# wonjune-kang/llm-speech-summarization

Measured on AMD Instinct MI355X. Metric: generated tokens/s of end-to-end generate_audio_response steps (encode + prefill + 256-token greedy decode), HuBERT-large -> Llama-3.2-3B; audio-sec/s reported beside it, encoder stage alone and in the pipeline, higher is better.
Workload: dtype bf16

## Files before the change

include/speechllm.h:

```cpp
#ifndef SPEECHLLM_H
#define SPEECHLLM_H

#include <stddef.h>
#include <stdint.h>

#ifdef __cplusplus
extern "C" {
#endif

typedef void* sl_stream;

enum sl_dtype { SL_F32 = 0, SL_BF16 = 1, SL_F16 = 2 };
enum sl_status {
  SL_OK = 0,
  SL_ERR_ARG = -1,
  SL_ERR_LAUNCH = -2,
  SL_ERR_UNSUPPORTED = -3
};
enum sl_act { SL_ACT_NONE = 0, SL_ACT_GELU = 1, SL_ACT_SILU_MUL = 2, SL_ACT_ROPE_KV = 3 };
enum sl_w_layout { SL_W_ROWMAJOR = 0, SL_W_PACKED = 1 };
#define SL_W_PACKED_E4M3 2

const char* sl_last_error(void);
#define SL_ABI_VERSION 7
// ... 11 lines not shown
  int32_t dtype, act, out_f32, w_layout;
} sl_gemm_args;
int sl_gemm(const sl_gemm_args* a, sl_stream stream);

int sl_pack_weight(const void* src, int64_t ld_src, void* dst, int32_t N, int32_t K, int32_t dtype, sl_stream stream);

size_t sl_w8_image_bytes(int32_t N, int32_t K);
int sl_pack_weight_e4m3(const void* src, int64_t ld_src, void* dst, int32_t N, int32_t K, int32_t dtype, sl_stream stream);
int sl_pack_weight_e4m3_host(const void* src, int64_t ld_src, void* dst, int32_t N, int32_t K, int32_t dtype);
int32_t sl_w8_max_rows(void);

typedef struct {
  int32_t fuse_rms; float rms_eps;
  const float* rope_cos; const float* rope_sin;
  const int32_t* tok_pos; const int32_t* tok_seq;
  void* k_cache; void* v_cache;
  int32_t n_heads, n_kv_heads, max_ctx, reserved;
  void* split_ws; size_t split_ws_bytes;
  const float* rstd_in; float* rstd_out;
  void* norm_out; const void* norm_gain;
} sl_gemm_fused;
size_t sl_gemm_split_workspace_bytes(int32_t M, int32_t N, int32_t K, int32_t dtype);
int32_t sl_gemm_split_count(int32_t M, int32_t N, int32_t K, int32_t dtype);
int sl_gemm_fused_decode(const sl_gemm_args* a, const sl_gemm_fused* fx, sl_stream stream);

typedef struct {
  int32_t trans_a, trans_w, residual_f32, w_mod;
  void* aux_out;
  const int64_t* groups;
  int32_t groups_ext, reserved;
  float* amax_val; int32_t* amax_idx;
  const float* ln_mr; const float* ln_u; const float* ln_c; float* stats_out;
  void* sk_ws; size_t sk_ws_bytes;
  int32_t post_op, post_reserved;
  float drop_p; float post_reserved_f;
  uint64_t drop_seed;
  int64_t drop_ld;
  const void* post_in; int64_t post_ld;
  float* colsum_out;
  int32_t* deferred_splits;
} sl_gemm_ex_args;
enum { SL_POST_NONE = 0, SL_POST_DROPOUT = 1, SL_POST_GELU_BWD = 2, SL_POST_SILU_MUL_BWD = 3 };
int sl_gemm_ex(const sl_gemm_args* a, const sl_gemm_ex_args* ex, sl_stream stream);
size_t sl_gemm_streamk_workspace_bytes(void);
int32_t sl_gemm_ln_fold_ok(int32_t M, int32_t N, int32_t K, int32_t dtype);
int sl_layernorm_fold_build(const void* W, const void* gain, const void* beta, const void* bias, void* Wf, float* u, float* c, int32_t N,
// ... 411 lines not shown
```

llm-speech-summarization_amd/_lib.py:

```python
from __future__ import annotations

import ctypes as C
import os

import torch

_HERE = os.path.dirname(os.path.abspath(__file__))
LIB_PATH = (os.environ.get("SL_LIB_PATH") if os.environ.get("SL_DEV") == "1" else None) or os.path.join(_HERE, "libspeechllm.so")

SL_F32, SL_BF16, SL_F16 = 0, 1, 2
KV_MODEL_DTYPE, KV_FP8_E4M3 = 0, 1
ACT_NONE, ACT_GELU, ACT_SILU_MUL, ACT_ROPE_KV = 0, 1, 2, 3
POST_NONE, POST_DROPOUT, POST_GELU_BWD, POST_SILU_MUL_BWD = 0, 1, 2, 3
W_ROWMAJOR, W_PACKED, W_PACKED_E4M3 = 0, 1, 2
WDEC_MODEL_DTYPE, WDEC_E4M3 = 0, 1
COMM_ID_BYTES = 128
MAX_DECODE_BATCH = 2048

c_i32, c_i64, c_f32, c_vp, c_sz = C.c_int32, C.c_int64, C.c_float, C.c_void_p, C.c_size_t


class SpeechLLMError(RuntimeError):
    pass

# ... 163 lines not shown
    "sl_device_arch": (c_i32, [C.c_char_p, c_i32]),
    "sl_tuning_reload": (c_i32, []),
    "sl_decode_graph_cache_clear": (c_i32, []),
    "sl_gemm": (c_i32, [C.POINTER(GemmArgs), c_vp]),
    "sl_gemm_streamk_workspace_bytes": (C.c_size_t, []),
    "sl_layernorm_fold_build": (c_i32, [c_vp, c_vp, c_vp, c_vp, c_vp, c_vp, c_vp, c_i32, c_i32, c_i32, c_vp]),
    "sl_weight_norm_bwd": (c_i32, [c_vp, c_vp, c_vp, c_vp, c_vp, c_vp, c_i32, c_i32, c_i32, c_vp]),
    "sl_weight_norm_bwd_workspace_bytes": (C.c_size_t, [c_i32]),
    "sl_comm_unique_id": (c_i32, [c_vp]),
    "sl_comm_init": (c_i32, [C.POINTER(c_vp), c_vp, c_i32, c_i32]),
    "sl_allreduce_sum": (c_i32, [c_vp, c_vp, c_i64, c_i32, c_vp]),
    "sl_comm_destroy": (c_i32, [c_vp]),
    "sl_comm_abort": (c_i32, [c_vp]),
    "sl_comm_rank": (c_i32, [c_vp]),
    "sl_comm_world": (c_i32, [c_vp]),
    "sl_pack_weight": (c_i32, [c_vp, c_i64, c_vp, c_i32, c_i32, c_i32, c_vp]),
    "sl_w8_image_bytes": (c_sz, [c_i32, c_i32]),
    "sl_pack_weight_e4m3": (c_i32, [c_vp, c_i64, c_vp, c_i32, c_i32, c_i32, c_vp]),
    "sl_pack_weight_e4m3_host": (c_i32, [c_vp, c_i64, c_vp, c_i32, c_i32, c_i32]),
    "sl_w8_max_rows": (c_i32, []),
    "sl_gemm_fused_decode": (c_i32, [C.POINTER(GemmArgs), C.POINTER(GemmFused), c_vp]),
    "sl_gemm_split_workspace_bytes": (c_sz, [c_i32, c_i32, c_i32, c_i32]),
    "sl_gemm_split_count": (c_i32, [c_i32, c_i32, c_i32, c_i32]),
    "sl_attn_decode_workspace_bytes": (c_sz, [c_i32, c_i32, c_i32, c_i32]),
    "sl_attn_decode_split": (c_i32, [c_vp, c_i64, c_vp, c_vp, c_vp, c_vp, c_vp, c_i32, c_i32, c_i32, c_i32, c_i32, c_f32, c_i32, c_vp]),
    "sl_gemm_ex": (c_i32, [C.POINTER(GemmArgs), C.POINTER(GemmEx), c_vp]),
    "sl_gemm_ln_fold_ok": (c_i32, [c_i32, c_i32, c_i32, c_i32]),
    "sl_layernorm_stats_finalize": (c_i32, [c_vp, c_i32, c_i64, c_i32, c_f32, c_vp, c_vp]),
    "sl_layernorm_stats": (c_i32, [c_vp, c_i64, c_i32, c_f32, c_vp, c_i32, c_vp]),
    "sl_gelu_bwd": (c_i32, [c_vp, c_vp, c_vp, c_i64, c_i32, c_vp]),
    "sl_axpby": (c_i32, [c_vp, c_vp, c_f32, c_f32, c_i64, c_i32, c_vp]),
    "sl_adamw_blocks": (C.c_size_t, [c_i64]),
    "sl_adamw_step": (c_i32, [c_vp, c_vp, c_i32, c_i64, C.c_double, C.c_double, C.c_double, C.c_double, C.c_double, c_i64, c_vp]),
    "sl_attn_dropout_bwd": (c_i32, [c_vp, c_vp, c_vp, c_i64, c_i32, c_vp, c_i32, c_vp, c_i32, c_i32, c_i32, c_f32, C.c_uint64, c_i32, c_vp]),
    "sl_transpose_pad": (c_i32, [c_vp, c_i64, c_vp, c_i64, c_i32, c_i32, c_i32, c_i32, c_vp]),
    "sl_dropout": (c_i32, [c_vp, c_vp, c_vp, c_i64, c_f32, C.c_uint64, c_i32, c_vp]),
    "sl_silu_mul": (c_i32, [c_vp, c_vp, c_i64, c_i32, c_i32, c_vp]),
    "sl_silu_mul_bwd": (c_i32, [c_vp, c_vp, c_vp, c_i64, c_i32, c_i32, c_vp]),
    "sl_rope_inplace": (c_i32, [c_vp, c_vp, c_vp, c_vp, c_i64, c_i32, c_i32, c_i32, c_i32, c_i32, c_vp]),
    "sl_layernorm_bwd": (c_i32, [c_vp, c_vp, c_vp, c_vp, c_vp, c_vp, c_vp, c_i64, c_i32, c_f32, c_i32, c_i32, c_vp]),
    "sl_layernorm_bwd_ws_bytes": (c_sz, [c_i64, c_i32]),
    "sl_layernorm_bwd_ws": (c_i32, [c_vp, c_vp, c_vp, c_vp, c_vp, c_vp, c_vp, c_i64, c_i32, c_f32, c_i32, c_i32, c_vp, c_sz, c_vp]),
    "sl_rmsnorm_bwd": (c_i32, [c_vp, c_vp, c_vp, c_vp, c_i64, c_i32, c_f32, c_i32, c_vp]),
    "sl_colsum": (c_i32, [c_vp, c_i64, c_vp, c_i64, c_i32, c_i32, c_vp]),
    "sl_softmax_rows": (c_i32, [c_vp, c_vp, c_i64, c_i32, c_i32, c_i64, c_f32, c_i32, c_i32, c_vp]),
    "sl_softmax_bwd": (c_i32, [c_vp, c_vp, c_vp, c_i64, c_i32, c_i64, c_f32, c_i32, c_vp]),
# ... 168 lines not shown
```

llm-speech-summarization_amd/csrc/api.hip:

```cpp
#include <stdarg.h>
#include <stdlib.h>

#include <atomic>
#include <mutex>

#include "common.h"

static thread_local char g_err[512] = "";

void sl_set_error(const char* fmt, ...) {
  va_list ap;
  va_start(ap, fmt);
  vsnprintf(g_err, sizeof(g_err), fmt, ap);
  va_end(ap);
}

extern "C" const char* sl_last_error(void) { return g_err; }

extern "C" int sl_version(void) { return SL_ABI_VERSION; }

extern "C" int sl_kv_quantize_e4m3_host(const float* x, uint8_t* out, int64_t n) {
  SL_CHECK_ARG(x != nullptr && out != nullptr && n >= 0, "sl_kv_quantize_e4m3_host: bad arguments");
  for (int64_t i = 0; i < n; ++i) out[i] = (uint8_t)sl_q8_e4m3(x[i]);
  return 0;
// ... 56 lines not shown
  e.prefill_prune_last = env_int("SL_PREFILL_PRUNE_LAST", 1);
  e.gemm_ko = env_int("SL_GEMM_KO", 0);
  { const char* sp = getenv("SL_GEMM_STAMP_PTR"); e.gemm_stamp_ptr = (sp && sp[0]) ? strtoull(sp, nullptr, 16) : 0ull; }
  const char* g = getenv("SL_DISABLE_GLDS");
  e.disable_glds = (g && g[0] == '1') ? 1 : ((g && g[0] == '2') ? 2 : 0);
  e.direct_epilogue = env_int("SL_DIRECT_EPILOGUE", 0);
  e.gemm_gm = env_int("SL_GEMM_GM", 8);
  e.attn_full_min = env_int("SL_ATTN_FULL_MIN", 32);
  e.attn_force_split = getenv("SL_ATTN_FORCE_SPLIT") != nullptr;
  { const int ks = env_int("SL_ATTN_DECODE_KS", 128); e.attn_decode_ks = (ks == 64 || ks == 65) ? ks : 128; }
  e.attn_split_merge = env_int("SL_ATTN_SPLIT_MERGE", -1);
  e.attn_generic = env_int("SL_ATTN_GENERIC", 0);
  e.attn_qt = env_int("SL_ATTN_QT", 0);
  e.norm_single_row = env_int("SL_NORM_SINGLE_ROW", 0);
  e.no_ln_fold = env_int("SL_NO_LN_FOLD", 0);
  e.no_swap_epilogue = env_int("SL_NO_SWAP_EPILOGUE", 0);
  e.gemm_log = env_int("SL_GEMM_LOG", 0);
  e.no_wgrad_stream = env_int("SL_NO_WGRAD_STREAM", 0);
  e.stream_splits = e.stream_nwv = e.stream_mt = 0;
  e.stream_nl = env_int("SL_STREAM_NL", 0);
  e.stream_wide = env_int("SL_STREAM_WIDE", 1);
  e.stream_wsplits = env_int("SL_STREAM_WSPLITS", 0);
  e.stream_fixup = env_int("SL_STREAM_FIXUP", 0);
  const char* sc = getenv("SL_STREAM_CFG");
  if (sc && sc[0]) {
    int sp = 0, nwv = 0, mt = 0;
    const int n = sscanf(sc, "%d,%d,%d", &sp, &nwv, &mt);
    if (n >= 2) {
      if (sp >= 1 && sp <= 64) e.stream_splits = sp;
      if (nwv == 2 || nwv == 4) e.stream_nwv = nwv;
    }
    if (n == 3 && (mt == 8 || mt == 16)) e.stream_mt = mt;
  }
  return &e;
}

const SlEnv& sl_env() {
  const SlEnv* e = g_env.load(std::memory_order_acquire);
  if (!e) {
    std::lock_guard<std::mutex> lk(g_env_mu);
    e = g_env.load(std::memory_order_relaxed);
    if (!e) {
      e = env_load();
      g_env.store(e, std::memory_order_release);
    }
  }
// ... 17 lines not shown
```

llm-speech-summarization_amd/csrc/common.h:

```cpp
#pragma once
#include <hip/hip_runtime.h>
#include <stdint.h>
#include <stdio.h>
#include <string.h>

#include "../../include/speechllm.h"

void sl_set_error(const char* fmt, ...);

#define SL_CHECK_ARG(cond, ...)      \
  do {                               \
    if (!(cond)) {                   \
      sl_set_error(__VA_ARGS__);     \
      return SL_ERR_ARG;             \
    }                                \
  } while (0)

#define SL_CHECK_LAUNCH(what)                                                        \
  do {                                                                               \
    hipError_t e__ = hipGetLastError();                                              \
    if (e__ != hipSuccess) {                                                         \
      sl_set_error("%s: %s", what, hipGetErrorString(e__));                          \
      return SL_ERR_LAUNCH;                                                          \
    }                                                                                \
// ... 371 lines not shown
  int attn_split_merge;
  int attn_generic;
  int attn_qt;
  int norm_single_row;
  int no_ln_fold;
  int no_wgrad_stream;
  int gemm_log;
  int no_swap_epilogue;
  int decode_tiled;
  int prefill_share_prefix;
  int prefill_prune_last;
  int skinny_alt;
  int tt_max_splits;
  int lnbwd_nw;
  int wgrad_tr;
  int split_k;
  int stream_k;
  int gemm_ko;
  unsigned long long gemm_stamp_ptr;
  int stream_splits, stream_nwv, stream_mt;
  int stream_wide;
  int stream_wsplits;
  int stream_fixup;
  int stream_nl;
};
const SlEnv& sl_env();

#define SL_TRANSPOSE_BATCH 64
struct SlTransposeRec {
  const void* x; void* y;
  int64_t ldx, ldy;
  int32_t rows, cols, ld_out, tiles_r;
};
struct SlTransposeBatch {
  SlTransposeRec rec[SL_TRANSPOSE_BATCH];
  int32_t first_block[SL_TRANSPOSE_BATCH];
  int32_t n, pad;
};
int sl_transpose_pad_batch_impl(const SlTransposeRec* recs, int n, int32_t dtype, sl_stream stream);
int sl_family_rows(int rows);
int sl_family_pin(int rows);
struct SlFamilyPin {
  int prev;
  explicit SlFamilyPin(int rows) : prev(sl_family_pin(rows)) {}
  ~SlFamilyPin() { sl_family_pin(prev); }
};
// ... 1 lines not shown
```

llm-speech-summarization_amd/csrc/gemm_stream.hip:

```cpp
#include <type_traits>
#include <stdlib.h>

#include <atomic>

#include "gemm_internal.h"

struct StreamX {
  float* part;
  float* part_ss;
  int splits, sps;
  int np;
  int* cnt;
  float* ss_part;
};

__device__ __forceinline__ void st_sc1_16(float* ptr, const f32x4& v) {
  asm volatile("global_store_dwordx4 %0, %1, off sc1" ::"v"(ptr), "v"(v) : "memory");
}
__device__ __forceinline__ void ld_sc1_16(f32x4& v, const float* ptr) {
  asm volatile("global_load_dwordx4 %0, %1, off sc1" : "=v"(v) : "v"(ptr) : "memory");
}
__device__ __forceinline__ void vm_drain16(f32x4 (&v)[16]) {
  asm volatile("s_waitcnt vmcnt(0)"
               : "+v"(v[0]), "+v"(v[1]), "+v"(v[2]), "+v"(v[3]), "+v"(v[4]), "+v"(v[5]), "+v"(v[6]), "+v"(v[7]), "+v"(v[8]), "+v"(v[9]), "+v"(v[10]),
// ... 278 lines not shown
#pragma unroll
    for (int d = 0; d < D - 1; ++d)
      if (n_full + d < n_it) stage(d, n_full + d);
    if constexpr (FUSE) {
#pragma unroll
      for (int j = 0; j < NSS; ++j) {
        const int t = j * NWV + wn;
        if (t < MT && (r >> 2) == q) ssl[t * 16 + r] = ssacc[j][r & 3];
      }
    }
  }
  __syncthreads();
  if (wave >= NWV) return;

  float ssum[MT];
#pragma unroll
  for (int t = 0; t < MT; ++t) {
    ssum[t] = 0.f;
    if (fuse) ssum[t] = ssl[t * 16 + r];
  }
  stream_finish<T, MT, ACT, RF>(p, sx, s, acc, ssum, fuse, m0, sp, fi0, nfrag, nb == 0 && wn == 0, q, r);
}

template <typename T, int ACT>
__global__ __launch_bounds__(768) void gemm_stream_wide_kernel(GemmP p, SkinnyX sx, StreamX s) {
  constexpr int VEC = Vec16<T>::VEC;
  constexpr int KSTEP = MMA<T>::KSTEP;
  constexpr int CW = 8;
  constexpr int MTW = 4, RFW = 4;
  constexpr int BM = 256, BF = 8;
  constexpr int SLAB_X = BM * TROWB, SLAB_W = BF * 2 * 1024, SLOT = SLAB_X + SLAB_W;
  constexpr int NSLOT = 3;
  constexpr int NDMA = 12;
  extern __shared__ __attribute__((aligned(16))) unsigned char smem[];
  __shared__ int fx_last[2];
  __shared__ float fx_ss[4][2][64];

  const int tid = threadIdx.x, lane = tid & 63;
  const int wave = __builtin_amdgcn_readfirstlane(tid >> 6);
  const int r = lane & 15, q = lane >> 4;
  const int mblocks = (p.M + BM - 1) / BM;
  const int nfrag = (p.N + 15) >> 4;
  const int xj = blockIdx.x >> 3, nb = (xj / mblocks) * 8 + (blockIdx.x & 7);
  if (nb * BF >= nfrag) return;
  const int mblock = xj % mblocks;
  const int m0 = mblock * BM;
  const int sp = blockIdx.z;
  const int nks = p.K / KSTEP;
  const int g_lo = sp * s.sps;
  const int g_hi = min(nks >> 1, g_lo + s.sps);
  const int n_it = g_hi - g_lo;
  const int g_last = g_hi - 1;
  const int wm = (wave >> 1) & 3, wn = wave & 1;
  const int mw = m0 + wm * 64, fi0 = nb * BF + wn * RFW;

  f32x4 acc[RFW][MTW];
  float ssum[MTW];
#pragma unroll
  for (int t = 0; t < MTW; ++t) {
    ssum[t] = 0.f;
#pragma unroll
    for (int f = 0; f < RFW; ++f) acc[f][t] = f32x4{0.f, 0.f, 0.f, 0.f};
  }

  if (wave >= CW) {
    const int lw = wave - CW;
    const T* A = (const T*)p.A;
    const T* W = (const T*)p.W;
    const int ch = (lane & 7) ^ ((lane >> 3) & 7);
    const T* gx[8];
#pragma unroll
    for (int i = 0; i < 8; ++i) {
      int xr_ = m0 + lw * 64 + (lane >> 3) + 8 * i; xr_ = xr_ < p.M ? xr_ : p.M - 1;
      gx[i] = A + (int64_t)xr_ * p.lda + ch * VEC;
    }
    const T* gw[2];
#pragma unroll
    for (int f = 0; f < 2; ++f) {
      int fi = nb * BF + lw * 2 + f; fi = fi < nfrag ? fi : nfrag - 1;
      gw[f] = W + (int64_t)fi * nks * (64 * VEC) + lane * VEC;
    }
    unsigned char* xbase = smem + lw * (64 * TROWB);
    unsigned char* wbase = smem + SLAB_X + lw * (2 * 2 * 1024);
    auto dma = [&](int it) {
      int stg = g_lo + it; stg = stg < g_last ? stg : g_last;
      const int so = (it % NSLOT) * SLOT;
#pragma unroll
      for (int i = 0; i < 8; ++i)
        __builtin_amdgcn_global_load_lds((glb_ptr_t)(gx[i] + (int64_t)stg * (2 * KSTEP)), (lds_ptr_t)(xbase + so + i * 1024), 16, 0, 0);
#pragma unroll
      for (int f = 0; f < 2; ++f)
#pragma unroll
        for (int s2 = 0; s2 < 2; ++s2)
          __builtin_amdgcn_global_load_lds((glb_ptr_t)(gw[f] + (int64_t)(stg * 2 + s2) * (64 * VEC)), (lds_ptr_t)(wbase + so + (f * 2 + s2) * 1024), 16, 0, 0);
    };
    dma(0);
    dma(1);
    asm volatile("s_waitcnt vmcnt(%0)" ::"n"(NDMA) : "memory");
    __builtin_amdgcn_s_barrier();
    for (int it = 0; it < n_it; ++it) {
      dma(it + 2);
      asm volatile("s_waitcnt vmcnt(%0)" ::"n"(NDMA) : "memory");
      __builtin_amdgcn_s_barrier();
    }
    asm volatile("s_waitcnt vmcnt(0)" ::: "memory");
  } else {
    uint4 fx[2][MTW], fw[2][RFW];
    auto rd = [&](int it, int s2, int set) {
      const unsigned char* sl_ = smem + (it % NSLOT) * SLOT;
#pragma unroll
      for (int t = 0; t < MTW; ++t) fx[set][t] = *(const uint4*)(sl_ + lds_off(wm * 64 + t * 16 + r, s2 * 4 + q));
#pragma unroll
      for (int f = 0; f < RFW; ++f) fw[set][f] = *(const uint4*)(sl_ + SLAB_X + ((wn * RFW + f) * 2 + s2) * 1024 + lane * 16);
    };
    auto mma = [&](int set) {
#pragma unroll
      for (int t = 0; t < MTW; ++t)
#pragma unroll
        for (int f = 0; f < RFW; ++f) MMA<T>::step(acc[f][t], fw[set][f], fx[set][t]);
      if constexpr (sizeof(T) == 2) {
#pragma unroll
        for (int i = 0; i < MTW + RFW; ++i) {
          __builtin_amdgcn_sched_group_barrier(0x008, 2, 0);
          __builtin_amdgcn_sched_group_barrier(0x100, 1, 0);
        }
      }
    };
    __builtin_amdgcn_s_barrier();
    rd(0, 0, 0);
    for (int it = 0; it < n_it; ++it) {
      __builtin_amdgcn_sched_barrier(0);
      rd(it, 1, 1);
      mma(0);
      __builtin_amdgcn_sched_barrier(0);
      asm volatile("s_waitcnt lgkmcnt(0)" ::: "memory");
      __builtin_amdgcn_s_barrier();
      rd(it + 1, 0, 0);
      mma(1);
      __builtin_amdgcn_sched_barrier(0);
    }
    stream_finish<T, MTW, ACT, RFW>(p, sx, s, acc, ssum, false, mw, sp, fi0, nfrag, false, q, r);
  }
  if (!(s.splits > 1 && s.cnt)) return;

  const bool cw = wave < CW;
  const int tile = nb * mblocks + mblock;
  asm volatile("s_waitcnt vmcnt(0)" ::: "memory");
  __builtin_amdgcn_s_barrier();
  if (tid == 0) {
    const int old = atomicAdd(&s.cnt[tile], 1);
    fx_last[0] = old == s.splits - 1;
    if (old == s.splits - 1) s.cnt[tile] = 0;
  }
  __builtin_amdgcn_s_barrier();
  if (!fx_last[0]) return;
  bool rowstat = false;
  if constexpr (ACT == SL_ACT_NONE) rowstat = sx.rstd_out != nullptr;
  if (cw) {
#pragma unroll
    for (int t = 0; t < MTW; ++t)
#pragma unroll
      for (int f = 0; f < RFW; ++f) acc[f][t] = f32x4{0.f, 0.f, 0.f, 0.f};
    for (int sp2 = 0; sp2 < s.splits; ++sp2) {
      f32x4 v[MTW * RFW];
#pragma unroll
// ... 57 lines not shown
      const int m = m0 + tid;
      if (m < p.M)
        __hip_atomic_store(&s.ss_part[(int64_t)nb * p.M + m], fx_ss[tid >> 6][0][tid & 63] + fx_ss[tid >> 6][1][tid & 63], __ATOMIC_RELAXED,
                           __HIP_MEMORY_SCOPE_AGENT);
    }
    asm volatile("s_waitcnt vmcnt(0)" ::: "memory");
    __builtin_amdgcn_s_barrier();
    if (tid == 0) {
      const int old = atomicAdd(&s.cnt[1024 + mblock], 1);
      fx_last[1] = old == nbv - 1;
      if (old == nbv - 1) s.cnt[1024 + mblock] = 0;
    }
    __builtin_amdgcn_s_barrier();
    if (!fx_last[1]) return;
    if (tid < 256) {
      const int m = m0 + tid;
      if (m < p.M) {
        float t = 0.f;
        for (int j = 0; j < nbv; ++j) t += __hip_atomic_load(&s.ss_part[(int64_t)j * p.M + m], __ATOMIC_RELAXED, __HIP_MEMORY_SCOPE_AGENT);
        sx.rstd_out[m] = rsqrtf(t / (float)p.N + sx.eps);
      }
    }
  }
}

template <int UN, int NCH, bool PAIRS>
__device__ __forceinline__ void reduce_add_splits(const float* rec, int64_t split_stride, int sp0, const uint32_t (&voff)[NCH], f32x4 (&a4)[NCH],
                                                  f32x4 (&b4)[NCH]) {
  f32x4 va[NCH][UN], vb[NCH][UN];
#pragma unroll
  for (int u = 0; u < UN; ++u) {
    const float* row = rec + (int64_t)(sp0 + u) * split_stride;
#pragma unroll
    for (int j = 0; j < NCH; ++j) {
      va[j][u] = *(const f32x4*)(row + voff[j]);
      if constexpr (PAIRS) vb[j][u] = *(const f32x4*)(row + voff[j] + 16);
    }
  }
#pragma unroll
  for (int u = 0; u < UN; ++u)
#pragma unroll
    for (int j = 0; j < NCH; ++j) {
      a4[j] += va[j][u];
      if constexpr (PAIRS) b4[j] += vb[j][u];
    }
}
// ... 212 lines not shown
            const uint2 w = *(const uint2*)gain;
            const f32x2_t lo = unpack2<T>(w.x), hi = unpack2<T>(w.y);
            g4[0] = lo.x; g4[1] = lo.y; g4[2] = hi.x; g4[3] = hi.y;
          } else {
#pragma unroll
            for (int i = 0; i < 4; ++i) g4[i] = to_f32(gain[i]);
          }
        } else {
#pragma unroll
          for (int i = 0; i < 4; ++i) g4[i] = to_f32(gain[i]);
        }
#pragma unroll
        for (int i = 0; i < 4; ++i) o[i] = g4[i] * norm_round<T>(kept[j][i], rstd);
        if constexpr (sizeof(T) == 2) *(uint2*)dst = make_uint2(pack2<T>(o[0], o[1]), pack2<T>(o[2], o[3]));
        else *(f32x4*)dst = f32x4{o[0], o[1], o[2], o[3]};
      } else {
        for (int i = 0; i < 4 && col0[j] + i < (uint32_t)p.N; ++i)
          dst[i] = from_f32<T>(to_f32(gain[i]) * norm_round<T>(kept[j][i], rstd));
      }
    }
  }
}

struct StreamCfg { int mt, splits, nwv, d, nl; int wide, wsplits; };

static StreamCfg stream_cfg(int M, int N, int K, int kstep, bool have_ws, int dtype) {
  StreamCfg c;
  c.mt = M <= 32 ? 2 : (M <= 64 ? 4 : 8);
  const int nfrag = (N + 15) / 16;
  const int nst = K / (2 * kstep);
  c.d = 4;
  c.nl = sl_env().stream_nl ? sl_env().stream_nl : 1;
  const int sp_env = sl_env().stream_splits, nwv_env = sl_env().stream_nwv;
  if (sl_env().stream_mt && M > 64) c.mt = sl_env().stream_mt;
  const int mblocks = (M + c.mt * 16 - 1) / (c.mt * 16);
  c.nwv = ((nfrag + 7) / 8 * mblocks >= 512 || M > 128) && c.mt <= 8 ? 4 : 2;
  if (nwv_env && c.mt <= 8) c.nwv = nwv_env;
  const int base = mblocks * ((nfrag + c.nwv * 2 - 1) / (c.nwv * 2));
  int splits = 1;
  if (have_ws) {
    splits = 208 / base;
    const int max_splits = nst / 4 > 0 ? nst / 4 : 1;
    if (splits > max_splits) splits = max_splits;
    if (splits > 16) splits = 16;
    if (splits < 1) splits = 1;
  }
  if (sp_env && (have_ws || sp_env == 1)) splits = sp_env < nst ? sp_env : nst;
  c.splits = splits;
  c.wide = 0; c.wsplits = 1;
  if (sl_is16(dtype) && M > 384 && sl_env().stream_wide != 0) {
    const int wbase = ((M + 255) / 256) * ((nfrag + 7) / 8);
    if (wbase >= 128 || sl_env().stream_wide == 2) {
      c.wide = 1;
    }
    if (wbase < 128 && have_ws) {
      int ws_ = 240 / wbase;
      const int max_ws = nst / 6 > 0 ? nst / 6 : 1;
      if (ws_ > max_ws) ws_ = max_ws;
      if (ws_ > 8) ws_ = 8;
      if (sl_env().stream_wsplits) ws_ = sl_env().stream_wsplits < nst ? sl_env().stream_wsplits : nst;
      if (ws_ > 1) { c.wide = 1; c.wsplits = ws_; }
    }
  }
  return c;
}

static size_t stream_ws_header(int M) { return 8192 + (((size_t)32 * M * sizeof(float) + 255) & ~(size_t)255); }

int sl_gemm_stream_splits(int M, int N, int K, int dtype) {
  const StreamCfg c = stream_cfg(sl_family_rows(M), N, K, dtype == SL_F32 ? 16 : 32, true, dtype);
  return c.wide ? c.wsplits : c.splits;
}

size_t sl_gemm_stream_ws_bytes(int M, int N, int K, int dtype) {
  const size_t np = (size_t)((N + 15) / 16) * 16;
  const StreamCfg c = stream_cfg(sl_family_rows(M), N, K, dtype == SL_F32 ? 16 : 32, true, dtype);
  const int most = c.wide && c.wsplits > c.splits ? c.wsplits : c.splits;
  size_t splits = most > 1 ? (size_t)most : 0;
  return stream_ws_header(M) + splits * ((size_t)M * np + (size_t)M) * sizeof(float) + 256;
}

template <typename T, int ACT>
static int launch_stream_reduce(GemmP& p, const SkinnyX& sx, const StreamX& s, hipStream_t st) {
  if (s.splits <= 1) return 0;
  constexpr bool PAIRS = (ACT == SL_ACT_SILU_MUL || sl_act_is_rope_kv(ACT));
  const int nfrag = (p.N + 15) / 16;
  const int64_t nunits = PAIRS ? (nfrag + 1) / 2 : nfrag;
  const int64_t threads = (int64_t)p.M * nunits * 4;
  if constexpr (ACT == SL_ACT_NONE) {
    if (sx.rstd_out) {
      const uintptr_t al = sizeof(T) == 2 ? 7 : 15;
      const bool fast = !p.bias && p.res && !p.res_f32 && !p.out_f32 && !sx.fuse_rms && !sx.rstd_in && !(p.N & 3) && !(p.ldc & 3) && !(p.ldr & 3) &&
                        !((uintptr_t)p.C & al) && !((uintptr_t)p.res & al) && (!sx.norm_out || (!((uintptr_t)sx.norm_out & al) && !((uintptr_t)sx.norm_gain & al)));
      const int nch = (nfrag * 4 + 255) / 256;
#define SL_ROWSTAT_LAUNCH(NCH_)                                                                                                              \
  if (fast) hipLaunchKernelGGL((gemm_stream_reduce_rowstat_kernel<T, NCH_, true>), dim3(p.M), dim3(256), 0, st, p, sx, s);                   \
  else hipLaunchKernelGGL((gemm_stream_reduce_rowstat_kernel<T, NCH_, false>), dim3(p.M), dim3(256), 0, st, p, sx, s)
      if (nch <= 1) { SL_ROWSTAT_LAUNCH(1); }
      else if (nch == 2) { SL_ROWSTAT_LAUNCH(2); }
// ... 50 lines not shown
    default: return launch_stream_mt<T, 16, ACT>(p, sx, s, c, st);
  }
}

template <typename T>
static int stream_typed(GemmP& p, const SkinnyX& sx, int act, const StreamX& s, const StreamCfg& c, hipStream_t st) {
  switch (act) {
    case SL_ACT_NONE: return launch_stream<T, SL_ACT_NONE>(p, sx, s, c, st);
    case SL_ACT_SILU_MUL: return launch_stream<T, SL_ACT_SILU_MUL>(p, sx, s, c, st);
    case SL_ACT_ROPE_KV:
      if constexpr (sizeof(T) == 2) { if (sx.kv8) return launch_stream<T, SL_ACT_ROPE_KV8>(p, sx, s, c, st); }
      return launch_stream<T, SL_ACT_ROPE_KV>(p, sx, s, c, st);
  }
  sl_set_error("sl_gemm: packed weights are not built with act %d for M > 16 streaming", act);
  return SL_ERR_UNSUPPORTED;
}

static bool stream_wide_ok(const SkinnyX& sx, int act, const StreamCfg& c, bool have_ws) {
  if (!c.wide || (sx.fuse_rms != 0 && sx.rstd_in == nullptr)) return false;
  if (act != SL_ACT_NONE && act != SL_ACT_SILU_MUL && act != SL_ACT_ROPE_KV) return false;
  return c.wsplits == 1 || have_ws;
}

template <typename T, int ACT>
static int launch_stream_wide_act(GemmP& p, const SkinnyX& sx, const StreamX& s, hipStream_t st) {
  const int nfrag = (p.N + 15) / 16, mblocks = (p.M + 255) / 256, nblocks = (nfrag + 7) / 8;
  constexpr int LDS_BYTES = 3 * (256 * TROWB + 8 * 2 * 1024);
  dim3 grid((nblocks + 7) / 8 * 8 * mblocks, 1, s.splits);
  static std::atomic<uint64_t> attr_set{0};
  int devid = 0;
  SL_HIP(hipGetDevice(&devid));
  if (devid < 0 || devid >= 64 || !((attr_set.load(std::memory_order_relaxed) >> devid) & 1)) {
    SL_HIP(hipFuncSetAttribute((const void*)gemm_stream_wide_kernel<T, ACT>, hipFuncAttributeMaxDynamicSharedMemorySize, LDS_BYTES));
    if (devid >= 0 && devid < 64) attr_set.fetch_or(1ull << devid, std::memory_order_relaxed);
  }
  hipLaunchKernelGGL((gemm_stream_wide_kernel<T, ACT>), grid, dim3(768), LDS_BYTES, st, p, sx, s);
  SL_CHECK_LAUNCH("gemm_stream_wide");
  if (s.cnt) return 0;
  return launch_stream_reduce<T, ACT>(p, sx, s, st);
}

template <typename T>
static int launch_stream_wide(GemmP& p, const SkinnyX& sx, int act, const StreamX& s, hipStream_t st) {
  switch (act) {
    case SL_ACT_SILU_MUL: return launch_stream_wide_act<T, SL_ACT_SILU_MUL>(p, sx, s, st);
    case SL_ACT_ROPE_KV:
      if constexpr (sizeof(T) == 2) { if (sx.kv8) return launch_stream_wide_act<T, SL_ACT_ROPE_KV8>(p, sx, s, st); }
      return launch_stream_wide_act<T, SL_ACT_ROPE_KV>(p, sx, s, st);
    default: return launch_stream_wide_act<T, SL_ACT_NONE>(p, sx, s, st);
  }
}

int sl_gemm_stream_launch(GemmP& p, const SkinnyX& sx, int dtype, int act, void* split_ws, size_t split_ws_bytes, hipStream_t st) {
  const int kstep = dtype == SL_F32 ? 16 : 32;
  SL_CHECK_ARG(p.K % (2 * kstep) == 0, "sl_gemm: streaming path needs K %% %d == 0 (K=%d)", 2 * kstep, p.K);
  StreamCfg c = stream_cfg(sl_family_rows(p.M), p.N, p.K, kstep, split_ws != nullptr, dtype);
  StreamX s;
  const bool wide = stream_wide_ok(sx, act, c, split_ws != nullptr);
  if (wide) c.splits = c.wsplits;

  s.np = (p.N + 15) / 16 * 16;
  const size_t per_split = ((size_t)p.M * s.np + (size_t)p.M) * sizeof(float);
  const size_t hdr = stream_ws_header(p.M);
  split_ws_bytes = (split_ws && split_ws_bytes > hdr) ? split_ws_bytes - hdr : 0;
  if (c.splits > 1 && (size_t)c.splits * per_split > split_ws_bytes) c.splits = (int)(split_ws_bytes / per_split);
  if (c.splits < 1) c.splits = 1;
  const int nst = p.K / (2 * kstep);
  s.sps = (nst + c.splits - 1) / c.splits;
  s.splits = (nst + s.sps - 1) / s.sps;
  c.splits = s.splits;
  SL_CHECK_ARG(sx.norm_out == nullptr || sx.rstd_out != nullptr, "sl_gemm: norm_out comes from the pass that forms rstd_out (pass both)");
  if (sx.rstd_out) {
    SL_CHECK_ARG(act == SL_ACT_NONE && (p.N + 15) / 16 * 4 <= 1024 && s.splits > 1,
                 "sl_gemm: rstd_out needs the plain epilogue, N <= 4096 and a K-split (splits=%d; see sl_gemm_split_count)", s.splits);
  }
  s.part = split_ws ? (float*)((unsigned char*)split_ws + hdr) : nullptr;
  s.part_ss = s.part ? s.part + (size_t)s.splits * p.M * s.np : nullptr;
  s.cnt = nullptr; s.ss_part = nullptr;
  if (wide && s.splits > 1 && sl_env().stream_fixup != 0 && sx.norm_out == nullptr) {
    const int nbv = ((p.N + 15) / 16 + 7) / 8, mbl = (p.M + 255) / 256;
    if (nbv * mbl <= 1024 && mbl <= 64 && (sx.rstd_out == nullptr || nbv <= 32)) {
      s.cnt = (int*)split_ws;
      s.ss_part = (float*)((unsigned char*)split_ws + 8192);
    }
  }
  if (dtype == SL_F32) return stream_typed<float>(p, sx, act, s, c, st);
  if (dtype == SL_F16) {
    if (wide) return launch_stream_wide<f16_t>(p, sx, act, s, st);
    return stream_typed<f16_t>(p, sx, act, s, c, st);
  }
  if (wide) return launch_stream_wide<bf16_t>(p, sx, act, s, st);
  return stream_typed<bf16_t>(p, sx, act, s, c, st);
}
```

llm-speech-summarization_amd/csrc/runtime.hip:

```cpp
#include <cmath>
#include <vector>

#include "common.h"
#include "gemm_internal.h"

int sl_attn_decode_impl(const void* q, int64_t q_stride, const void* k_cache, const void* v_cache, void* out, const int32_t* ctx_len,
                        int ctx_add, int32_t B, int32_t n_heads, int32_t n_kv, int32_t D, int32_t max_ctx, float scale, int32_t dtype,
                        hipStream_t st);
int sl_greedy_select_impl(const float* logits, int32_t B, int32_t V, const int32_t* eos_ids, int32_t n_eos, int32_t pad_id,
                          int32_t use_eos, int32_t advance_ctx, int32_t* unfinished, int32_t* ctx_len, int32_t* gen_count,
                          int32_t* finish_len, int32_t* next_ids, int32_t* out_ids, int32_t max_new, hipStream_t st, const int32_t* row_limit);
int sl_greedy_select_partial_impl(const float* amax_val, const int32_t* amax_idx, int32_t n_groups, int32_t B, const int32_t* eos_ids, int32_t n_eos,
                                  int32_t pad_id, int32_t use_eos, int32_t advance_ctx, int32_t* unfinished, int32_t* ctx_len, int32_t* gen_count,
                                  int32_t* finish_len, int32_t* next_ids, int32_t* out_ids, int32_t max_new, hipStream_t st, const int32_t* row_limit);
int sl_sample_select_impl(const float* logits, int32_t B, int32_t V, float temperature, int32_t top_k, float top_p, uint64_t seed,
                          const int32_t* eos_ids, int32_t n_eos, int32_t pad_id, int32_t use_eos, int32_t advance_ctx, int32_t* unfinished,
                          int32_t* ctx_len, int32_t* gen_count, int32_t* finish_len, int32_t* next_ids, int32_t* out_ids, int32_t max_new,
                          int32_t* choice_ws, hipStream_t st, const int32_t* row_limit, const int32_t* row_ids);

int sl_logits_opts_check(const char* who, const sl_logits_opts* lp, int max_new_tokens);
int sl_logits_process_impl(float* logits, int32_t rows, int32_t V, const int32_t* hist, const int32_t* hist_odd, int64_t hist_ld, const int32_t* hist_len,
                           const int32_t* unfinished, const sl_logits_opts* lp, const int32_t* eos_ids_host, int32_t n_eos, int32_t log_softmax,
                           float* scratch, hipStream_t st);

// ... 996 lines not shown
    if (smp)
      return sl_sample_select_impl(logits, B, m->vocab, smp->temperature, smp->top_k, smp->top_p, smp->seed, eos_ids_host, n_eos, pad_id, use_eos, advance_ctx,
                                   unfinished, ctx_len, gen_count, finish_len, next_ids, out_ids, max_new_tokens, choice, s_, row_limit_arg, row_id);
    return sl_greedy_select_impl(logits, B, m->vocab, eos_ids_host, n_eos, pad_id, use_eos, advance_ctx, unfinished, ctx_len, gen_count, finish_len, next_ids,
                                 out_ids, max_new_tokens, s_, row_limit_arg);
  };
  SL_TRY(select(B0, 0, st));
  SL_HIP(hipEventRecord(ev[1], st));

  const int pin_rows = (o->compact && use_eos && sl_env().compact_pin) ? B0 : 0;
  auto graph_for = [&](int B, hipGraphExec_t* exec_out) -> int {
    SlFamilyPin pin(pin_rows);
    LlamaWs w;
    llama_carve(m, B, B, scratch, scratch_bytes, w);
    if (w.split && w.split_bytes >= 8192) SL_HIP(hipMemsetAsync(w.split, 0, 8192, st));
    SL_TRY(sl_attn_decode_split_zero_counters(w.part, B, m->n_heads, m->n_kv_heads, kv->max_ctx, st));
    hipLaunchKernelGGL(iota_kernel, dim3((B + 255) / 256), dim3(256), 0, st, w.tok_seq, B);
    SL_CHECK_LAUNCH("iota");
    DecodeGraphKey key;
    memset(&key, 0, sizeof(key));
    key.model = m; key.layers = m->layers; key.w0 = m->n_layers > 0 ? m->layers[0].wqkv_dec : nullptr; key.lm = m->lm_head_dec ? m->lm_head_dec : m->lm_head;
    key.embed = m->embed; key.kc = kv->k_cache; key.vc = kv->v_cache; key.ws = workspace; key.ws_bytes = workspace_bytes;
    key.B = B; key.B0 = B0; key.max_new = max_new_tokens; key.use_eos = use_eos; key.n_eos = n_eos; key.pad = pad_id; key.max_ctx = kv->max_ctx;
    key.slots = kv->slots; key.shared_prefix = kv->shared_prefix; key.dtype = m->dtype; key.n_layers = m->n_layers; key.vocab = m->vocab; key.fused = m->dec_fused_norm | (sl_env().decode_tiled << 8) | ((sl_env().attn_decode_ks & 127) << 9) | ((pin_rows ? 1 : 0) << 16) | ((sl_env().decode_prefetch ? 1 : 0) << 17) | ((kv->reserved & 3) << 18) | ((m->reserved & 3) << 20);
    key.limits = row_limit_arg ? 1 : 0;
    key.content = model_content_hash(m);
    SL_HIP(hipGetDevice(&key.device));
    for (int i = 0; i < n_eos && i < 8; ++i) key.eos[i] = eos_ids_host[i];
    if (smp) { key.sample = 1; key.temperature = smp->temperature; key.top_k = smp->top_k; key.top_p = smp->top_p; key.seed = smp->seed; }
    if (lp.on) { key.lp_penalty = lp.o.repetition_penalty; key.lp_ngram = lp.o.no_repeat_ngram_size; key.lp_min_new = lp.o.min_new_tokens; }
    hipGraphExec_t exec = decode_graph_lookup(key);
    if (!exec) {
      hipGraph_t graph = nullptr;
      static thread_local hipStream_t cap_by_dev[SL_MAX_DEVICES] = {};
      SL_CHECK_ARG(key.device >= 0 && key.device < SL_MAX_DEVICES, "sl_generate: device index %d", key.device);
      hipStream_t& cap = cap_by_dev[key.device];
      if (!cap) SL_HIP(hipStreamCreateWithFlags(&cap, hipStreamNonBlocking));
      SL_HIP(hipStreamBeginCapture(cap, hipStreamCaptureModeThreadLocal));
      const bool top1 = !smp && !lp.on && decode_fuses_argmax(m, B);
      DecodePrefetch pf;
      static thread_local hipStream_t cap2_by_dev[SL_MAX_DEVICES] = {};
      static thread_local hipEvent_t pev_by_dev[SL_MAX_DEVICES] = {};
      if (sl_env().decode_prefetch && B <= sl_env().stream_min_m && m->dtype == SL_BF16) {
        hipStream_t& cap2 = cap2_by_dev[key.device];
        hipEvent_t& pev = pev_by_dev[key.device];
        if (!cap2) SL_HIP(hipStreamCreateWithFlags(&cap2, hipStreamNonBlocking));
        if (!pev) SL_HIP(hipEventCreateWithFlags(&pev, hipEventDisableTiming));
// ... 432 lines not shown
```

Measured before the change: 68690.

## Add 128-row wide streaming GEMM tile shapes for plain and RoPE/KV epilogues

Generalizes the wide streaming GEMM kernel over a shape template, adding 128-row tiles with 12 or 10 N-fragments per block alongside the original 256x8 shape. The DMA layout, wave mapping and scheduling hints are parameterized to match. By default the 10-fragment shape is picked only for RoPE/KV GEMMs with about 897-1024 rows where the grid divides evenly, aiming for better CU fill and less padding waste. The split-K in-kernel fixup is limited to the original shape, so the new shapes fall back to a separate reduce launch.

```diff
diff --git a/include/speechllm.h b/include/speechllm.h
--- a/include/speechllm.h
+++ b/include/speechllm.h
@@ -57,6 +57,7 @@
 } sl_gemm_fused;
 size_t sl_gemm_split_workspace_bytes(int32_t M, int32_t N, int32_t K, int32_t dtype);
 int32_t sl_gemm_split_count(int32_t M, int32_t N, int32_t K, int32_t dtype);
+int32_t sl_gemm_stream_shape(int32_t M, int32_t N, int32_t K, int32_t dtype, int32_t act);
 int sl_gemm_fused_decode(const sl_gemm_args* a, const sl_gemm_fused* fx, sl_stream stream);
 
 typedef struct {
diff --git a/llm-speech-summarization_amd/_lib.py b/llm-speech-summarization_amd/_lib.py
--- a/llm-speech-summarization_amd/_lib.py
+++ b/llm-speech-summarization_amd/_lib.py
@@ -209,6 +209,7 @@
     "sl_gemm_fused_decode": (c_i32, [C.POINTER(GemmArgs), C.POINTER(GemmFused), c_vp]),
     "sl_gemm_split_workspace_bytes": (c_sz, [c_i32, c_i32, c_i32, c_i32]),
     "sl_gemm_split_count": (c_i32, [c_i32, c_i32, c_i32, c_i32]),
+    "sl_gemm_stream_shape": (c_i32, [c_i32, c_i32, c_i32, c_i32, c_i32]),
     "sl_attn_decode_workspace_bytes": (c_sz, [c_i32, c_i32, c_i32, c_i32]),
     "sl_attn_decode_split": (c_i32, [c_vp, c_i64, c_vp, c_vp, c_vp, c_vp, c_vp, c_i32, c_i32, c_i32, c_i32, c_i32, c_f32, c_i32, c_vp]),
     "sl_gemm_ex": (c_i32, [C.POINTER(GemmArgs), C.POINTER(GemmEx), c_vp]),
diff --git a/llm-speech-summarization_amd/csrc/api.hip b/llm-speech-summarization_amd/csrc/api.hip
--- a/llm-speech-summarization_amd/csrc/api.hip
+++ b/llm-speech-summarization_amd/csrc/api.hip
@@ -102,6 +102,8 @@
   e.stream_wide = env_int("SL_STREAM_WIDE", 1);
   e.stream_wsplits = env_int("SL_STREAM_WSPLITS", 0);
   e.stream_fixup = env_int("SL_STREAM_FIXUP", 0);
+  e.stream_shape = env_int("SL_STREAM_SHAPE", 1);
+  if (e.stream_shape < 0 || e.stream_shape > 2) e.stream_shape = 1;
   const char* sc = getenv("SL_STREAM_CFG");
   if (sc && sc[0]) {
     int sp = 0, nwv = 0, mt = 0;
diff --git a/llm-speech-summarization_amd/csrc/common.h b/llm-speech-summarization_amd/csrc/common.h
--- a/llm-speech-summarization_amd/csrc/common.h
+++ b/llm-speech-summarization_amd/csrc/common.h
@@ -417,6 +417,7 @@
   int stream_wide;
   int stream_wsplits;
   int stream_fixup;
+  int stream_shape;
   int stream_nl;
 };
 const SlEnv& sl_env();
diff --git a/llm-speech-summarization_amd/csrc/gemm_stream.hip b/llm-speech-summarization_amd/csrc/gemm_stream.hip
--- a/llm-speech-summarization_amd/csrc/gemm_stream.hip
+++ b/llm-speech-summarization_amd/csrc/gemm_stream.hip
@@ -324,19 +324,32 @@
   stream_finish<T, MT, ACT, RF>(p, sx, s, acc, ssum, fuse, m0, sp, fi0, nfrag, nb == 0 && wn == 0, q, r);
 }
 
-template <typename T, int ACT>
-__global__ __launch_bounds__(768) void gemm_stream_wide_kernel(GemmP p, SkinnyX sx, StreamX s) {
+template <int SHAPE> struct WideShape;
+template <> struct WideShape<0> { static constexpr int BM = 256, BF = 8, WM = 4, WN = 2, RFW = 4; };
+template <> struct WideShape<12> { static constexpr int BM = 128, BF = 12, WM = 2, WN = 4, RFW = 3; };
+template <> struct WideShape<10> { static constexpr int BM = 128, BF = 10, WM = 2, WN = 5, RFW = 2; };
+template <int SHAPE> constexpr int wide_threads() { return 64 * (WideShape<SHAPE>::WM * WideShape<SHAPE>::WN + 4); }
+template <int SHAPE> constexpr int wide_lds_bytes() { return 3 * (WideShape<SHAPE>::BM * TROWB + WideShape<SHAPE>::BF * 2 * 1024); }
+
+template <typename T, int ACT, int SHAPE>
+__device__ __forceinline__ void stream_wide_block(const GemmP& p, const SkinnyX& sx, const StreamX& s) {
+  typedef WideShape<SHAPE> WS;
   constexpr int VEC = Vec16<T>::VEC;
   constexpr int KSTEP = MMA<T>::KSTEP;
-  constexpr int CW = 8;
-  constexpr int MTW = 4, RFW = 4;
-  constexpr int BM = 256, BF = 8;
+  constexpr int WN = WS::WN;
+  constexpr int CW = WS::WM * WN;
+  constexpr int MTW = 4, RFW = WS::RFW;
+  constexpr int BM = WS::BM, BF = WS::BF;
   constexpr int SLAB_X = BM * TROWB, SLAB_W = BF * 2 * 1024, SLOT = SLAB_X + SLAB_W;
   constexpr int NSLOT = 3;
-  constexpr int NDMA = 12;
+  constexpr int XRL = BM / 4, NXD = XRL / 8;
+  constexpr int NWD = BF * 2 / 4;
+  constexpr int NDMA = NXD + NWD;
+  constexpr bool PAIRS = (ACT == SL_ACT_SILU_MUL || sl_act_is_rope_kv(ACT));
+  static_assert(WS::WM * MTW * 16 == BM && WN * RFW == BF && (BF * 2) % 4 == 0 && XRL % 8 == 0, "block shape");
+  static_assert(!PAIRS || RFW % 2 == 0, "pair epilogues need both fragments of a pair in one wave");
+  static_assert(SHAPE == 0 || !(ACT == SL_ACT_SILU_MUL), "the 128-row shapes are instantiated for the plain and the RoPE / KV epilogues");
   extern __shared__ __attribute__((aligned(16))) unsigned char smem[];
-  __shared__ int fx_last[2];
-  __shared__ float fx_ss[4][2][64];
 
   const int tid = threadIdx.x, lane = tid & 63;
   const int wave = __builtin_amdgcn_readfirstlane(tid >> 6);
@@ -353,7 +366,7 @@
   const int g_hi = min(nks >> 1, g_lo + s.sps);
   const int n_it = g_hi - g_lo;
   const int g_last = g_hi - 1;
-  const int wm = (wave >> 1) & 3, wn = wave & 1;
+  const int wm = (wave / WN) % WS::WM, wn = wave % WN;
   const int mw = m0 + wm * 64, fi0 = nb * BF + wn * RFW;
 
   f32x4 acc[RFW][MTW];
@@ -370,31 +383,30 @@
     const T* A = (const T*)p.A;
     const T* W = (const T*)p.W;
     const int ch = (lane & 7) ^ ((lane >> 3) & 7);
-    const T* gx[8];
-#pragma unroll
-    for (int i = 0; i < 8; ++i) {
-      int xr_ = m0 + lw * 64 + (lane >> 3) + 8 * i; xr_ = xr_ < p.M ? xr_ : p.M - 1;
+    const T* gx[NXD];
+#pragma unroll
+    for (int i = 0; i < NXD; ++i) {
+      int xr_ = m0 + lw * XRL + (lane >> 3) + 8 * i; xr_ = xr_ < p.M ? xr_ : p.M - 1;
       gx[i] = A + (int64_t)xr_ * p.lda + ch * VEC;
     }
-    const T* gw[2];
-#pragma unroll
-    for (int f = 0; f < 2; ++f) {
-      int fi = nb * BF + lw * 2 + f; fi = fi < nfrag ? fi : nfrag - 1;
-      gw[f] = W + (int64_t)fi * nks * (64 * VEC) + lane * VEC;
-    }
-    unsigned char* xbase = smem + lw * (64 * TROWB);
-    unsigned char* wbase = smem + SLAB_X + lw * (2 * 2 * 1024);
+    const T* gw[NWD];
+#pragma unroll
+    for (int j = 0; j < NWD; ++j) {
+      const int c = lw * NWD + j;
+      int fi = nb * BF + (c >> 1); fi = fi < nfrag ? fi : nfrag - 1;
+      gw[j] = W + (int64_t)fi * nks * (64 * VEC) + lane * VEC + (c & 1) * (64 * VEC);
+    }
+    unsigned char* xbase = smem + lw * (XRL * TROWB);
+    unsigned char* wbase = smem + SLAB_X + lw * (NWD * 1024);
     auto dma = [&](int it) {
       int stg = g_lo + it; stg = stg < g_last ? stg : g_last;
       const int so = (it % NSLOT) * SLOT;
 #pragma unroll
-      for (int i = 0; i < 8; ++i)
+      for (int i = 0; i < NXD; ++i)
         __builtin_amdgcn_global_load_lds((glb_ptr_t)(gx[i] + (int64_t)stg * (2 * KSTEP)), (lds_ptr_t)(xbase + so + i * 1024), 16, 0, 0);
 #pragma unroll
-      for (int f = 0; f < 2; ++f)
-#pragma unroll
-        for (int s2 = 0; s2 < 2; ++s2)
-          __builtin_amdgcn_global_load_lds((glb_ptr_t)(gw[f] + (int64_t)(stg * 2 + s2) * (64 * VEC)), (lds_ptr_t)(wbase + so + (f * 2 + s2) * 1024), 16, 0, 0);
+      for (int j = 0; j < NWD; ++j)
+        __builtin_amdgcn_global_load_lds((glb_ptr_t)(gw[j] + (int64_t)(stg * 2) * (64 * VEC)), (lds_ptr_t)(wbase + so + j * 1024), 16, 0, 0);
     };
     dma(0);
     dma(1);
@@ -421,9 +433,10 @@
 #pragma unroll
         for (int f = 0; f < RFW; ++f) MMA<T>::step(acc[f][t], fw[set][f], fx[set][t]);
       if constexpr (sizeof(T) == 2) {
+        constexpr int PER = (MTW * RFW) / (MTW + RFW) > 1 ? (MTW * RFW) / (MTW + RFW) : 1;
 #pragma unroll
         for (int i = 0; i < MTW + RFW; ++i) {
-          __builtin_amdgcn_sched_group_barrier(0x008, 2, 0);
+          __builtin_amdgcn_sched_group_barrier(0x008, PER, 0);
           __builtin_amdgcn_sched_group_barrier(0x100, 1, 0);
         }
       }
@@ -443,6 +456,9 @@
     }
     stream_finish<T, MTW, ACT, RFW>(p, sx, s, acc, ssum, false, mw, sp, fi0, nfrag, false, q, r);
   }
+  if constexpr (SHAPE == 0) {
+  __shared__ int fx_last[2];
+  __shared__ float fx_ss[4][2][64];
   if (!(s.splits > 1 && s.cnt)) return;
 
   const bool cw = wave < CW;
@@ -546,6 +562,16 @@
       }
     }
   }
+  }
+}
+
+template <typename T, int ACT>
+__global__ __launch_bounds__(768) void gemm_stream_wide_kernel(GemmP p, SkinnyX sx, StreamX s) {
+  stream_wide_block<T, ACT, 0>(p, sx, s);
+}
+template <typename T, int ACT, int SHAPE>
+__global__ __launch_bounds__(wide_threads<SHAPE>()) void gemm_stream_wide128_kernel(GemmP p, SkinnyX sx, StreamX s) {
+  stream_wide_block<T, ACT, SHAPE>(p, sx, s);
 }
 
 template <int UN, int NCH, bool PAIRS>
@@ -804,9 +830,9 @@
   }
 }
 
-struct StreamCfg { int mt, splits, nwv, d, nl; int wide, wsplits; };
-
-static StreamCfg stream_cfg(int M, int N, int K, int kstep, bool have_ws, int dtype) {
+struct StreamCfg { int mt, splits, nwv, d, nl; int wide, wsplits, shape; };
+
+static StreamCfg stream_cfg(int M, int N, int K, int kstep, bool have_ws, int dtype, int act) {
   StreamCfg c;
   c.mt = M <= 32 ? 2 : (M <= 64 ? 4 : 8);
   const int nfrag = (N + 15) / 16;
@@ -844,19 +870,31 @@
       if (ws_ > 1) { c.wide = 1; c.wsplits = ws_; }
     }
   }
+  c.shape = 0;
+  const int mode = sl_env().stream_shape;
+  const int bf = act == SL_ACT_NONE ? 12 : (sl_act_is_rope_kv(act) ? 10 : 0);
+  if (c.wide && mode != 0 && bf) {
+    if (mode == 2) c.shape = bf;
+    else if (bf == 10 && M > 896 && M <= 1024 && nfrag % bf == 0 && 8 * (nfrag / bf) * c.wsplits == 256) c.shape = bf;
+  }
   return c;
 }
 
 static size_t stream_ws_header(int M) { return 8192 + (((size_t)32 * M * sizeof(float) + 255) & ~(size_t)255); }
 
 int sl_gemm_stream_splits(int M, int N, int K, int dtype) {
-  const StreamCfg c = stream_cfg(sl_family_rows(M), N, K, dtype == SL_F32 ? 16 : 32, true, dtype);
+  const StreamCfg c = stream_cfg(sl_family_rows(M), N, K, dtype == SL_F32 ? 16 : 32, true, dtype, SL_ACT_NONE);
   return c.wide ? c.wsplits : c.splits;
+}
+
+extern "C" int32_t sl_gemm_stream_shape(int32_t M, int32_t N, int32_t K, int32_t dtype, int32_t act) {
+  if (M <= 0 || N <= 0 || K <= 0 || K % (dtype == SL_F32 ? 32 : 64) != 0) return 0;
+  return stream_cfg(sl_family_rows(M), N, K, dtype == SL_F32 ? 16 : 32, true, dtype, act).shape;
 }
 
 size_t sl_gemm_stream_ws_bytes(int M, int N, int K, int dtype) {
   const size_t np = (size_t)((N + 15) / 16) * 16;
-  const StreamCfg c = stream_cfg(sl_family_rows(M), N, K, dtype == SL_F32 ? 16 : 32, true, dtype);
+  const StreamCfg c = stream_cfg(sl_family_rows(M), N, K, dtype == SL_F32 ? 16 : 32, true, dtype, SL_ACT_NONE);
   const int most = c.wide && c.wsplits > c.splits ? c.wsplits : c.splits;
   size_t splits = most > 1 ? (size_t)most : 0;
   return stream_ws_header(M) + splits * ((size_t)M * np + (size_t)M) * sizeof(float) + 256;
@@ -953,39 +991,50 @@
   return c.wsplits == 1 || have_ws;
 }
 
-template <typename T, int ACT>
+template <typename T, int ACT, int SHAPE>
 static int launch_stream_wide_act(GemmP& p, const SkinnyX& sx, const StreamX& s, hipStream_t st) {
-  const int nfrag = (p.N + 15) / 16, mblocks = (p.M + 255) / 256, nblocks = (nfrag + 7) / 8;
-  constexpr int LDS_BYTES = 3 * (256 * TROWB + 8 * 2 * 1024);
+  typedef WideShape<SHAPE> WS;
+  const int nfrag = (p.N + 15) / 16, mblocks = (p.M + WS::BM - 1) / WS::BM, nblocks = (nfrag + WS::BF - 1) / WS::BF;
+  constexpr int LDS_BYTES = wide_lds_bytes<SHAPE>();
   dim3 grid((nblocks + 7) / 8 * 8 * mblocks, 1, s.splits);
   static std::atomic<uint64_t> attr_set{0};
   int devid = 0;
   SL_HIP(hipGetDevice(&devid));
+  const void* fn;
+  if constexpr (SHAPE == 0) fn = (const void*)gemm_stream_wide_kernel<T, ACT>;
+  else fn = (const void*)gemm_stream_wide128_kernel<T, ACT, SHAPE>;
   if (devid < 0 || devid >= 64 || !((attr_set.load(std::memory_order_relaxed) >> devid) & 1)) {
-    SL_HIP(hipFuncSetAttribute((const void*)gemm_stream_wide_kernel<T, ACT>, hipFuncAttributeMaxDynamicSharedMemorySize, LDS_BYTES));
+    SL_HIP(hipFuncSetAttribute(fn, hipFuncAttributeMaxDynamicSharedMemorySize, LDS_BYTES));
     if (devid >= 0 && devid < 64) attr_set.fetch_or(1ull << devid, std::memory_order_relaxed);
   }
-  hipLaunchKernelGGL((gemm_stream_wide_kernel<T, ACT>), grid, dim3(768), LDS_BYTES, st, p, sx, s);
-  SL_CHECK_LAUNCH("gemm_stream_wide");
-  if (s.cnt) return 0;
+  if constexpr (SHAPE == 0) {
+    hipLaunchKernelGGL((gemm_stream_wide_kernel<T, ACT>), grid, dim3(768), LDS_BYTES, st, p, sx, s);
+    SL_CHECK_LAUNCH("gemm_stream_wide");
+    if (s.cnt) return 0;
+  } else {
+    hipLaunchKernelGGL((gemm_stream_wide128_kernel<T, ACT, SHAPE>), grid, dim3(wide_threads<SHAPE>()), LDS_BYTES, st, p, sx, s);
+    SL_CHECK_LAUNCH("gemm_stream_wide128");
+  }
   return launch_stream_reduce<T, ACT>(p, sx, s, st);
 }
 
 template <typename T>
-static int launch_stream_wide(GemmP& p, const SkinnyX& sx, int act, const StreamX& s, hipStream_t st) {
+static int launch_stream_wide(GemmP& p, const SkinnyX& sx, int act, int shape, const StreamX& s, hipStream_t st) {
   switch (act) {
-    case SL_ACT_SILU_MUL: return launch_stream_wide_act<T, SL_ACT_SILU_MUL>(p, sx, s, st);
+    case SL_ACT_SILU_MUL: return launch_stream_wide_act<T, SL_ACT_SILU_MUL, 0>(p, sx, s, st);
     case SL_ACT_ROPE_KV:
-      if constexpr (sizeof(T) == 2) { if (sx.kv8) return launch_stream_wide_act<T, SL_ACT_ROPE_KV8>(p, sx, s, st); }
-      return launch_stream_wide_act<T, SL_ACT_ROPE_KV>(p, sx, s, st);
-    default: return launch_stream_wide_act<T, SL_ACT_NONE>(p, sx, s, st);
+      if constexpr (sizeof(T) == 2) {
+        if (sx.kv8) return shape == 10 ? launch_stream_wide_act<T, SL_ACT_ROPE_KV8, 10>(p, sx, s, st) : launch_stream_wide_act<T, SL_ACT_ROPE_KV8, 0>(p, sx, s, st);
+      }
+      return shape == 10 ? launch_stream_wide_act<T, SL_ACT_ROPE_KV, 10>(p, sx, s, st) : launch_stream_wide_act<T, SL_ACT_ROPE_KV, 0>(p, sx, s, st);
+    default: return shape == 12 ? launch_stream_wide_act<T, SL_ACT_NONE, 12>(p, sx, s, st) : launch_stream_wide_act<T, SL_ACT_NONE, 0>(p, sx, s, st);
   }
 }
 
 int sl_gemm_stream_launch(GemmP& p, const SkinnyX& sx, int dtype, int act, void* split_ws, size_t split_ws_bytes, hipStream_t st) {
   const int kstep = dtype == SL_F32 ? 16 : 32;
   SL_CHECK_ARG(p.K % (2 * kstep) == 0, "sl_gemm: streaming path needs K %% %d == 0 (K=%d)", 2 * kstep, p.K);
-  StreamCfg c = stream_cfg(sl_family_rows(p.M), p.N, p.K, kstep, split_ws != nullptr, dtype);
+  StreamCfg c = stream_cfg(sl_family_rows(p.M), p.N, p.K, kstep, split_ws != nullptr, dtype, act);
   StreamX s;
   const bool wide = stream_wide_ok(sx, act, c, split_ws != nullptr);
   if (wide) c.splits = c.wsplits;
@@ -1008,7 +1057,7 @@
   s.part = split_ws ? (float*)((unsigned char*)split_ws + hdr) : nullptr;
   s.part_ss = s.part ? s.part + (size_t)s.splits * p.M * s.np : nullptr;
   s.cnt = nullptr; s.ss_part = nullptr;
-  if (wide && s.splits > 1 && sl_env().stream_fixup != 0 && sx.norm_out == nullptr) {
+  if (wide && c.shape == 0 && s.splits > 1 && sl_env().stream_fixup != 0 && sx.norm_out == nullptr) {
     const int nbv = ((p.N + 15) / 16 + 7) / 8, mbl = (p.M + 255) / 256;
     if (nbv * mbl <= 1024 && mbl <= 64 && (sx.rstd_out == nullptr || nbv <= 32)) {
       s.cnt = (int*)split_ws;
@@ -1017,9 +1066,9 @@
   }
   if (dtype == SL_F32) return stream_typed<float>(p, sx, act, s, c, st);
   if (dtype == SL_F16) {
-    if (wide) return launch_stream_wide<f16_t>(p, sx, act, s, st);
+    if (wide) return launch_stream_wide<f16_t>(p, sx, act, c.shape, s, st);
     return stream_typed<f16_t>(p, sx, act, s, c, st);
   }
-  if (wide) return launch_stream_wide<bf16_t>(p, sx, act, s, st);
+  if (wide) return launch_stream_wide<bf16_t>(p, sx, act, c.shape, s, st);
   return stream_typed<bf16_t>(p, sx, act, s, c, st);
 }
diff --git a/llm-speech-summarization_amd/csrc/runtime.hip b/llm-speech-summarization_amd/csrc/runtime.hip
--- a/llm-speech-summarization_amd/csrc/runtime.hip
+++ b/llm-speech-summarization_amd/csrc/runtime.hip
@@ -1042,7 +1042,7 @@
     key.model = m; key.layers = m->layers; key.w0 = m->n_layers > 0 ? m->layers[0].wqkv_dec : nullptr; key.lm = m->lm_head_dec ? m->lm_head_dec : m->lm_head;
     key.embed = m->embed; key.kc = kv->k_cache; key.vc = kv->v_cache; key.ws = workspace; key.ws_bytes = workspace_bytes;
     key.B = B; key.B0 = B0; key.max_new = max_new_tokens; key.use_eos = use_eos; key.n_eos = n_eos; key.pad = pad_id; key.max_ctx = kv->max_ctx;
-    key.slots = kv->slots; key.shared_prefix = kv->shared_prefix; key.dtype = m->dtype; key.n_layers = m->n_layers; key.vocab = m->vocab; key.fused = m->dec_fused_norm | (sl_env().decode_tiled << 8) | ((sl_env().attn_decode_ks & 127) << 9) | ((pin_rows ? 1 : 0) << 16) | ((sl_env().decode_prefetch ? 1 : 0) << 17) | ((kv->reserved & 3) << 18) | ((m->reserved & 3) << 20);
+    key.slots = kv->slots; key.shared_prefix = kv->shared_prefix; key.dtype = m->dtype; key.n_layers = m->n_layers; key.vocab = m->vocab; key.fused = m->dec_fused_norm | (sl_env().decode_tiled << 8) | ((sl_env().attn_decode_ks & 127) << 9) | ((pin_rows ? 1 : 0) << 16) | ((sl_env().decode_prefetch ? 1 : 0) << 17) | ((kv->reserved & 3) << 18) | ((m->reserved & 3) << 20) | ((sl_env().stream_shape & 3) << 22);
     key.limits = row_limit_arg ? 1 : 0;
     key.content = model_content_hash(m);
     SL_HIP(hipGetDevice(&key.device));
```

After: 68520. About the same (-0.2%).
